# tongdaxu/VQ-VAE-from-Gaussian-VAE

Hardware: AMD Instinct MI355X
Metric: images/sec encode+quantize+decode, 256x256, codebook 2^16 (higher is better)
Workload: dtype f32

## Files before the change

vq-vae-from-gaussian-vae_amd/csrc/gq_wino_gemm.h:

```cpp
#pragma once
#include "gq_common.h"

namespace gqhip {

typedef _Float16 f16x8 __attribute__((ext_vector_type(8)));

struct WinoGemm2Params {
  const _Float16 *V2;
  const _Float16 *Wf;
  float *M;
  long tiles;
  int cin, cout, nnb;
  long mtiles;
  long ntile_total;
  long tiles_per_xcd;
};

__global__ __launch_bounds__(256, 2) void wino_gemm_f16x2_kernel(const WinoGemm2Params p) {
  constexpr int kPlane = 256 * 32 + 64, kChunk = 2 * kPlane, kStage = 2 * kChunk;
  __shared__ __attribute__((aligned(16))) unsigned char sA[2 * kStage];
  const int tid = threadIdx.x, lane = tid & 63, wave = __builtin_amdgcn_readfirstlane(tid >> 6);
  const int c = lane & 31, h = lane >> 5, wm = wave >> 1, wn = wave & 1;
  const long vb = blockIdx.x, kq = vb >> 3;
  const int nb = (int)(kq % p.nnb);
  const long tile = (vb & 7) * p.tiles_per_xcd + kq / p.nnb;
  if (tile >= p.ntile_total) return;
  const long pos = tile / p.mtiles, m0 = (tile % p.mtiles) * 256;
  const int cin = p.cin, nst = cin / 32;
  const int w8 = tid & 7, r0 = tid >> 3, pl = w8 >> 2, jc = (w8 >> 1) & 1, jh = w8 & 1;
  const _Float16 *src = p.V2 + ((pos * p.tiles + m0 + r0) * 2L * cin) + pl * cin + 16 * jc + 8 * jh;
  const int loff = jc * kChunk + pl * kPlane + r0 * 32 + 16 * (jh ^ ((r0 >> 3) & 1));
  const long rstride = 64L * cin;
  f16x8 st[8];
  auto issue = [&](int stage) {
#pragma unroll
    for (int i = 0; i < 8; ++i) st[i] = *reinterpret_cast<const f16x8 *>(src + i * rstride + stage * 32);
  };
  auto commit = [&](int buf) {
#pragma unroll
    for (int i = 0; i < 8; ++i) *reinterpret_cast<f16x8 *>(sA + buf * kStage + loff + i * 1024) = st[i];
  };
  f32x16 acc[4][2];
#pragma unroll
  for (int rr = 0; rr < 4; ++rr)
#pragma unroll
    for (int j = 0; j < 2; ++j)
      acc[rr][j] = f32x16{0.f, 0.f, 0.f, 0.f, 0.f, 0.f, 0.f, 0.f, 0.f, 0.f, 0.f, 0.f, 0.f, 0.f, 0.f, 0.f};
  const int aoff = (4 * wm) * 1024 + c * 32 + 16 * (h ^ ((c >> 3) & 1));
  const long wstep = (long)p.nnb * (512 * 16);
  const unsigned char *wbase = reinterpret_cast<const unsigned char *>(p.Wf) + pos * (cin / 16) * wstep +
                               (4 * nb + 2 * wn) * 128 * 16;
  const int wl = lane * 16;
  f16x8 b0[4], b1[4];
  auto load_b = [&](int ks, f16x8 (&dst)[4]) {
    const unsigned char *s = wbase + ks * wstep;
#pragma unroll
    for (int k = 0; k < 4; ++k) dst[k] = *reinterpret_cast<const f16x8 *>(s + k * 1024 + wl);
  };
  auto kstep = [&](const unsigned char *A, const f16x8 (&bq)[4]) {
#pragma unroll
    for (int rr = 0; rr < 4; ++rr) {
      const f16x8 ah = *reinterpret_cast<const f16x8 *>(A + aoff + rr * 1024);
      const f16x8 al = *reinterpret_cast<const f16x8 *>(A + aoff + rr * 1024 + kPlane);
#pragma unroll
      for (int j = 0; j < 2; ++j) {
        acc[rr][j] = __builtin_amdgcn_mfma_f32_32x32x16_f16(ah, bq[2 * j], acc[rr][j], 0, 0, 0);
        acc[rr][j] = __builtin_amdgcn_mfma_f32_32x32x16_f16(ah, bq[2 * j + 1], acc[rr][j], 0, 0, 0);
        acc[rr][j] = __builtin_amdgcn_mfma_f32_32x32x16_f16(al, bq[2 * j], acc[rr][j], 0, 0, 0);
      }
    }
  };
  const int nks = 2 * nst;
  load_b(0, b0);
  issue(0);
  commit(0);
  __syncthreads();
  for (int s = 0; s < nst; ++s) {
    const bool more = s + 1 < nst;
    const unsigned char *A = sA + (s & 1) * kStage;
    load_b(2 * s + 1, b1);
    if (more) issue(s + 1);
    kstep(A, b0);
    __builtin_amdgcn_sched_barrier(0);
    load_b(2 * s + 2 < nks ? 2 * s + 2 : nks - 1, b0);
    kstep(A + kChunk, b1);
    if (more) commit((s + 1) & 1);
    __builtin_amdgcn_sched_barrier(0);
    __syncthreads();
  }
  float *Mp = p.M + ((pos * p.tiles + m0 + 4 * wm * 32 + 4 * h) * (long)p.cout) + nb * 128 + c;
  const long cs = p.cout;
#pragma unroll
  for (int rr = 0; rr < 4; ++rr)
#pragma unroll
    for (int j = 0; j < 2; ++j) {
      float *base = Mp + (rr * 32L) * cs + (2 * wn + j) * 32;
#pragma unroll
      for (int r = 0; r < 16; ++r) base[(long)((r & 3) + 8 * (r >> 2)) * cs] = acc[rr][j][r];
    }
}

__global__ __launch_bounds__(512, 1) void wino_gemm_f16x2_w8_kernel(const WinoGemm2Params p) {
  constexpr int kPlane = 256 * 32 + 32, kChunk = 2 * kPlane, kStage = 4 * kChunk;
  static_assert(kChunk % 256 == 64 && kPlane % 256 == 32, "region stagger");
  __shared__ __attribute__((aligned(16))) unsigned char sA[2 * kStage];
  const int tid = threadIdx.x, lane = tid & 63, wave = __builtin_amdgcn_readfirstlane(tid >> 6);
  const int c = lane & 31, h = lane >> 5, wm = wave >> 2, wn = wave & 3;
  const long vb = blockIdx.x, kq = vb >> 3;
  const int nb = (int)(kq % p.nnb);
  const long tile = (vb & 7) * p.tiles_per_xcd + kq / p.nnb;
  if (tile >= p.ntile_total) return;
  const long pos = tile / p.mtiles, m0 = (tile % p.mtiles) * 256;
  const int cin = p.cin, nst = cin / 64;
  const int w16 = tid & 15, r0 = tid >> 4, pl = w16 >> 3, jc = (w16 >> 1) & 3, jh = w16 & 1;
  const _Float16 *src = p.V2 + ((pos * p.tiles + m0 + r0) * 2L * cin) + pl * cin + 16 * jc + 8 * jh;
  const int loff = jc * kChunk + pl * kPlane + r0 * 32 + 16 * (jh ^ ((r0 >> 3) & 1));
  const long rstride = 64L * cin;
  f16x8 st[8];
  auto issue = [&](int stage) {
#pragma unroll
    for (int i = 0; i < 8; ++i) st[i] = *reinterpret_cast<const f16x8 *>(src + i * rstride + stage * 64);
  };
  auto commit = [&](int buf) {
#pragma unroll
    for (int i = 0; i < 8; ++i) *reinterpret_cast<f16x8 *>(sA + buf * kStage + loff + i * 1024) = st[i];
  };
  f32x16 acc[4][2];
#pragma unroll
  for (int rr = 0; rr < 4; ++rr)
#pragma unroll
    for (int j = 0; j < 2; ++j)
      acc[rr][j] = f32x16{0.f, 0.f, 0.f, 0.f, 0.f, 0.f, 0.f, 0.f, 0.f, 0.f, 0.f, 0.f, 0.f, 0.f, 0.f, 0.f};
  const int aoff = (4 * wm) * 1024 + c * 32 + 16 * (h ^ ((c >> 3) & 1));
  const long wstep = (long)(p.cout / 32) * 2048;
  const unsigned char *wbase = reinterpret_cast<const unsigned char *>(p.Wf) + pos * (cin / 16) * wstep +
                               (8 * nb + 2 * wn) * 2048L;
  const int wl = lane * 16;
  const int nks = 4 * nst;
  f16x8 bA[4], bB[4], bC[4];
  auto load_b = [&](int ks, f16x8 (&dst)[4]) {
    const unsigned char *s = wbase + (long)(ks < nks ? ks : nks - 1) * wstep;
#pragma unroll
    for (int k = 0; k < 4; ++k) dst[k] = *reinterpret_cast<const f16x8 *>(s + k * 1024 + wl);
  };
  f16x8 ah, al, nh, nl;
  auto read_a = [&](const unsigned char *A, int u, f16x8 &oh, f16x8 &ol) {
    const unsigned char *q = A + (u >> 2) * kChunk + aoff + (u & 3) * 1024;
    oh = *reinterpret_cast<const f16x8 *>(q);
    ol = *reinterpret_cast<const f16x8 *>(q + kPlane);
  };
  auto mfma6 = [&](int rr, const f16x8 (&bq)[4]) {
#pragma unroll
    for (int j = 0; j < 2; ++j) {
      acc[rr][j] = __builtin_amdgcn_mfma_f32_32x32x16_f16(ah, bq[2 * j], acc[rr][j], 0, 0, 0);
      acc[rr][j] = __builtin_amdgcn_mfma_f32_32x32x16_f16(ah, bq[2 * j + 1], acc[rr][j], 0, 0, 0);
      acc[rr][j] = __builtin_amdgcn_mfma_f32_32x32x16_f16(al, bq[2 * j], acc[rr][j], 0, 0, 0);
    }
  };
  auto kstep = [&](const unsigned char *A, int ks4, const f16x8 (&bq)[4], bool last_of_stage) {
#pragma unroll
    for (int rr = 0; rr < 4; ++rr) {
      const int u = 4 * ks4 + rr;
      if (!(last_of_stage && rr == 3)) read_a(A, u + 1, nh, nl);
      __builtin_amdgcn_sched_barrier(0);
      mfma6(rr, bq);
      ah = nh;
      al = nl;
      __builtin_amdgcn_sched_barrier(0);
    }
  };
  load_b(0, bA);
  load_b(1, bB);
  issue(0);
  commit(0);
  __syncthreads();
  for (int s = 0; s < nst; ++s) {
    const bool more = s + 1 < nst;
    const unsigned char *A = sA + (s & 1) * kStage;
    read_a(A, 0, ah, al);
    load_b(4 * s + 2, bC);
    if (more) issue(s + 1);
    kstep(A, 0, bA, false);
    load_b(4 * s + 3, bA);
    kstep(A, 1, bB, false);
    load_b(4 * s + 4, bB);
    kstep(A, 2, bC, false);
    load_b(4 * s + 5, bC);
    kstep(A, 3, bA, true);
    if (more) commit((s + 1) & 1);
#pragma unroll
    for (int k = 0; k < 4; ++k) {
      bA[k] = bB[k];
      bB[k] = bC[k];
    }
    __builtin_amdgcn_sched_barrier(0);
    __syncthreads();
  }
  float *Mp = p.M + ((pos * p.tiles + m0 + 4 * wm * 32 + 4 * h) * (long)p.cout) + nb * 256 + c;
  const long cs = p.cout;
#pragma unroll
  for (int rr = 0; rr < 4; ++rr)
#pragma unroll
    for (int j = 0; j < 2; ++j) {
      float *base = Mp + (rr * 32L) * cs + (2 * wn + j) * 32;
#pragma unroll
      for (int r = 0; r < 16; ++r) base[(long)((r & 3) + 8 * (r >> 2)) * cs] = acc[rr][j][r];
    }
}

}
```

Before: 489.5.

## Switch Winograd GEMM kernels to 16x16x32 MFMA with transposed operands

```diff
diff --git a/vq-vae-from-gaussian-vae_amd/csrc/gq_wino_gemm.h b/vq-vae-from-gaussian-vae_amd/csrc/gq_wino_gemm.h
--- a/vq-vae-from-gaussian-vae_amd/csrc/gq_wino_gemm.h
+++ b/vq-vae-from-gaussian-vae_amd/csrc/gq_wino_gemm.h
@@ -20,7 +20,7 @@
   constexpr int kPlane = 256 * 32 + 64, kChunk = 2 * kPlane, kStage = 2 * kChunk;
   __shared__ __attribute__((aligned(16))) unsigned char sA[2 * kStage];
   const int tid = threadIdx.x, lane = tid & 63, wave = __builtin_amdgcn_readfirstlane(tid >> 6);
-  const int c = lane & 31, h = lane >> 5, wm = wave >> 1, wn = wave & 1;
+  const int c = lane & 15, g = lane >> 4, wm = wave >> 1, wn = wave & 1;
   const long vb = blockIdx.x, kq = vb >> 3;
   const int nb = (int)(kq % p.nnb);
   const long tile = (vb & 7) * p.tiles_per_xcd + kq / p.nnb;
@@ -40,64 +40,59 @@
 #pragma unroll
     for (int i = 0; i < 8; ++i) *reinterpret_cast<f16x8 *>(sA + buf * kStage + loff + i * 1024) = st[i];
   };
-  f32x16 acc[4][2];
+  f32x4 acc[8][4];
 #pragma unroll
-  for (int rr = 0; rr < 4; ++rr)
+  for (int m = 0; m < 8; ++m)
 #pragma unroll
-    for (int j = 0; j < 2; ++j)
-      acc[rr][j] = f32x16{0.f, 0.f, 0.f, 0.f, 0.f, 0.f, 0.f, 0.f, 0.f, 0.f, 0.f, 0.f, 0.f, 0.f, 0.f, 0.f};
-  const int aoff = (4 * wm) * 1024 + c * 32 + 16 * (h ^ ((c >> 3) & 1));
+    for (int n = 0; n < 4; ++n) acc[m][n] = f32x4{0.f, 0.f, 0.f, 0.f};
+  const int aoff = (g >> 1) * kChunk + (8 * wm) * 512 + c * 32 + 16 * ((g & 1) ^ ((c >> 3) & 1));
   const long wstep = (long)p.nnb * (512 * 16);
   const unsigned char *wbase = reinterpret_cast<const unsigned char *>(p.Wf) + pos * (cin / 16) * wstep +
-                               (4 * nb + 2 * wn) * 128 * 16;
-  const int wl = lane * 16;
-  f16x8 b0[4], b1[4];
-  auto load_b = [&](int ks, f16x8 (&dst)[4]) {
-    const unsigned char *s = wbase + ks * wstep;
+                               (4 * nb + 2 * wn) * 128 * 16 + (g >> 1) * wstep + (32 * (g & 1) + c) * 16;
+  f16x8 wH[4], wN[4], wL[4];
+  auto load_w = [&](int ks, int plane, f16x8 (&dst)[4]) {
+    const unsigned char *s = wbase + (long)(ks < nst ? ks : nst - 1) * 2 * wstep + plane * 1024;
 #pragma unroll
-    for (int k = 0; k < 4; ++k) dst[k] = *reinterpret_cast<const f16x8 *>(s + k * 1024 + wl);
+    for (int n = 0; n < 4; ++n) dst[n] = *reinterpret_cast<const f16x8 *>(s + (n >> 1) * 2048 + (n & 1) * 256);
   };
-  auto kstep = [&](const unsigned char *A, const f16x8 (&bq)[4]) {
+  auto products = [&](const unsigned char *A, int plane) {
 #pragma unroll
-    for (int rr = 0; rr < 4; ++rr) {
-      const f16x8 ah = *reinterpret_cast<const f16x8 *>(A + aoff + rr * 1024);
-      const f16x8 al = *reinterpret_cast<const f16x8 *>(A + aoff + rr * 1024 + kPlane);
+    for (int m = 0; m < 8; ++m) {
+      const f16x8 a = *reinterpret_cast<const f16x8 *>(A + plane * kPlane + aoff + m * 512);
 #pragma unroll
-      for (int j = 0; j < 2; ++j) {
-        acc[rr][j] = __builtin_amdgcn_mfma_f32_32x32x16_f16(ah, bq[2 * j], acc[rr][j], 0, 0, 0);
-        acc[rr][j] = __builtin_amdgcn_mfma_f32_32x32x16_f16(ah, bq[2 * j + 1], acc[rr][j], 0, 0, 0);
-        acc[rr][j] = __builtin_amdgcn_mfma_f32_32x32x16_f16(al, bq[2 * j], acc[rr][j], 0, 0, 0);
+      for (int n = 0; n < 4; ++n) acc[m][n] = __builtin_amdgcn_mfma_f32_16x16x32_f16(wH[n], a, acc[m][n], 0, 0, 0);
+      if (plane == 0) {
+#pragma unroll
+        for (int n = 0; n < 4; ++n) acc[m][n] = __builtin_amdgcn_mfma_f32_16x16x32_f16(wL[n], a, acc[m][n], 0, 0, 0);
       }
     }
   };
-  const int nks = 2 * nst;
-  load_b(0, b0);
+  load_w(0, 0, wH);
+  load_w(0, 1, wL);
   issue(0);
   commit(0);
   __syncthreads();
   for (int s = 0; s < nst; ++s) {
     const bool more = s + 1 < nst;
     const unsigned char *A = sA + (s & 1) * kStage;
-    load_b(2 * s + 1, b1);
+    load_w(s + 1, 0, wN);
     if (more) issue(s + 1);
-    kstep(A, b0);
+    products(A, 0);
     __builtin_amdgcn_sched_barrier(0);
-    load_b(2 * s + 2 < nks ? 2 * s + 2 : nks - 1, b0);
-    kstep(A + kChunk, b1);
+    load_w(s + 1, 1, wL);
+    products(A, 1);
     if (more) commit((s + 1) & 1);
+#pragma unroll
+    for (int n = 0; n < 4; ++n) wH[n] = wN[n];
     __builtin_amdgcn_sched_barrier(0);
     __syncthreads();
   }
-  float *Mp = p.M + ((pos * p.tiles + m0 + 4 * wm * 32 + 4 * h) * (long)p.cout) + nb * 128 + c;
+  float *Mp = p.M + ((pos * p.tiles + m0 + 8 * wm * 16 + c) * (long)p.cout) + nb * 128 + wn * 64 + 4 * g;
   const long cs = p.cout;
 #pragma unroll
-  for (int rr = 0; rr < 4; ++rr)
+  for (int m = 0; m < 8; ++m)
 #pragma unroll
-    for (int j = 0; j < 2; ++j) {
-      float *base = Mp + (rr * 32L) * cs + (2 * wn + j) * 32;
-#pragma unroll
-      for (int r = 0; r < 16; ++r) base[(long)((r & 3) + 8 * (r >> 2)) * cs] = acc[rr][j][r];
-    }
+    for (int n = 0; n < 4; ++n) *reinterpret_cast<f32x4 *>(Mp + (m * 16L) * cs + n * 16) = acc[m][n];
 }
 
 __global__ __launch_bounds__(512, 1) void wino_gemm_f16x2_w8_kernel(const WinoGemm2Params p) {
@@ -105,7 +100,7 @@
   static_assert(kChunk % 256 == 64 && kPlane % 256 == 32, "region stagger");
   __shared__ __attribute__((aligned(16))) unsigned char sA[2 * kStage];
   const int tid = threadIdx.x, lane = tid & 63, wave = __builtin_amdgcn_readfirstlane(tid >> 6);
-  const int c = lane & 31, h = lane >> 5, wm = wave >> 2, wn = wave & 3;
+  const int c = lane & 15, g = lane >> 4, wm = wave >> 2, wn = wave & 3;
   const long vb = blockIdx.x, kq = vb >> 3;
   const int nb = (int)(kq % p.nnb);
   const long tile = (vb & 7) * p.tiles_per_xcd + kq / p.nnb;
@@ -125,87 +120,69 @@
 #pragma unroll
     for (int i = 0; i < 8; ++i) *reinterpret_cast<f16x8 *>(sA + buf * kStage + loff + i * 1024) = st[i];
   };
-  f32x16 acc[4][2];
+  f32x4 acc[8][4];
 #pragma unroll
-  for (int rr = 0; rr < 4; ++rr)
+  for (int m = 0; m < 8; ++m)
 #pragma unroll
-    for (int j = 0; j < 2; ++j)
-      acc[rr][j] = f32x16{0.f, 0.f, 0.f, 0.f, 0.f, 0.f, 0.f, 0.f, 0.f, 0.f, 0.f, 0.f, 0.f, 0.f, 0.f, 0.f};
-  const int aoff = (4 * wm) * 1024 + c * 32 + 16 * (h ^ ((c >> 3) & 1));
+    for (int n = 0; n < 4; ++n) acc[m][n] = f32x4{0.f, 0.f, 0.f, 0.f};
+  const int aoff = (g >> 1) * kChunk + (8 * wm) * 512 + c * 32 + 16 * ((g & 1) ^ ((c >> 3) & 1));
   const long wstep = (long)(p.cout / 32) * 2048;
   const unsigned char *wbase = reinterpret_cast<const unsigned char *>(p.Wf) + pos * (cin / 16) * wstep +
-                               (8 * nb + 2 * wn) * 2048L;
-  const int wl = lane * 16;
-  const int nks = 4 * nst;
-  f16x8 bA[4], bB[4], bC[4];
-  auto load_b = [&](int ks, f16x8 (&dst)[4]) {
-    const unsigned char *s = wbase + (long)(ks < nks ? ks : nks - 1) * wstep;
+                               (8 * nb + 2 * wn) * 2048L + (g >> 1) * wstep + (32 * (g & 1) + c) * 16;
+  const int nk32 = 2 * nst;
+  f16x8 wH0[4], wH1[4], wL[4], aq[4];
+  auto load_w = [&](int ks, int plane, f16x8 (&dst)[4]) {
+    const unsigned char *s = wbase + (long)(ks < nk32 ? ks : nk32 - 1) * 2 * wstep + plane * 1024;
 #pragma unroll
-    for (int k = 0; k < 4; ++k) dst[k] = *reinterpret_cast<const f16x8 *>(s + k * 1024 + wl);
+    for (int n = 0; n < 4; ++n) dst[n] = *reinterpret_cast<const f16x8 *>(s + (n >> 1) * 2048 + (n & 1) * 256);
   };
-  f16x8 ah, al, nh, nl;
-  auto read_a = [&](const unsigned char *A, int u, f16x8 &oh, f16x8 &ol) {
-    const unsigned char *q = A + (u >> 2) * kChunk + aoff + (u & 3) * 1024;
-    oh = *reinterpret_cast<const f16x8 *>(q);
-    ol = *reinterpret_cast<const f16x8 *>(q + kPlane);
+  auto read_a = [&](const unsigned char *A, int u, f16x8 &o) {
+    o = *reinterpret_cast<const f16x8 *>(A + (u >> 4) * 2 * kChunk + ((u >> 3) & 1) * kPlane + aoff + (u & 7) * 512);
   };
-  auto mfma6 = [&](int rr, const f16x8 (&bq)[4]) {
+  auto unit = [&](int u, const f16x8 &a, const f16x8 (&wh)[4], const f16x8 (&wl)[4]) {
+    const int m = u & 7;
 #pragma unroll
-    for (int j = 0; j < 2; ++j) {
-      acc[rr][j] = __builtin_amdgcn_mfma_f32_32x32x16_f16(ah, bq[2 * j], acc[rr][j], 0, 0, 0);
-      acc[rr][j] = __builtin_amdgcn_mfma_f32_32x32x16_f16(ah, bq[2 * j + 1], acc[rr][j], 0, 0, 0);
-      acc[rr][j] = __builtin_amdgcn_mfma_f32_32x32x16_f16(al, bq[2 * j], acc[rr][j], 0, 0, 0);
+    for (int n = 0; n < 4; ++n) acc[m][n] = __builtin_amdgcn_mfma_f32_16x16x32_f16(wh[n], a, acc[m][n], 0, 0, 0);
+    if (((u >> 3) & 1) == 0) {
+#pragma unroll
+      for (int n = 0; n < 4; ++n) acc[m][n] = __builtin_amdgcn_mfma_f32_16x16x32_f16(wl[n], a, acc[m][n], 0, 0, 0);
     }
   };
-  auto kstep = [&](const unsigned char *A, int ks4, const f16x8 (&bq)[4], bool last_of_stage) {
-#pragma unroll
-    for (int rr = 0; rr < 4; ++rr) {
-      const int u = 4 * ks4 + rr;
-      if (!(last_of_stage && rr == 3)) read_a(A, u + 1, nh, nl);
-      __builtin_amdgcn_sched_barrier(0);
-      mfma6(rr, bq);
-      ah = nh;
-      al = nl;
-      __builtin_amdgcn_sched_barrier(0);
-    }
-  };
-  load_b(0, bA);
-  load_b(1, bB);
+  load_w(0, 0, wH0);
+  load_w(0, 1, wL);
+  load_w(1, 0, wH1);
   issue(0);
   commit(0);
   __syncthreads();
   for (int s = 0; s < nst; ++s) {
     const bool more = s + 1 < nst;
     const unsigned char *A = sA + (s & 1) * kStage;
-    read_a(A, 0, ah, al);
-    load_b(4 * s + 2, bC);
+    read_a(A, 0, aq[0]);
+    read_a(A, 1, aq[1]);
+    read_a(A, 2, aq[2]);
     if (more) issue(s + 1);
-    kstep(A, 0, bA, false);
-    load_b(4 * s + 3, bA);
-    kstep(A, 1, bB, false);
-    load_b(4 * s + 4, bB);
-    kstep(A, 2, bC, false);
-    load_b(4 * s + 5, bC);
-    kstep(A, 3, bA, true);
+#pragma unroll
+    for (int u = 0; u < 32; ++u) {
+      if (u + 3 < 32) read_a(A, u + 3, aq[(u + 3) & 3]);
+      __builtin_amdgcn_sched_barrier(0);
+      if (u < 16) unit(u, aq[u & 3], wH0, wL);
+      else unit(u, aq[u & 3], wH1, wL);
+      __builtin_amdgcn_sched_barrier(0);
+      if (u == 7) load_w(2 * s + 1, 1, wL);
+      if (u == 15) load_w(2 * s + 2, 0, wH0);
+      if (u == 23) load_w(2 * s + 2, 1, wL);
+      if (u == 31) load_w(2 * s + 3, 0, wH1);
+    }
     if (more) commit((s + 1) & 1);
-#pragma unroll
-    for (int k = 0; k < 4; ++k) {
-      bA[k] = bB[k];
-      bB[k] = bC[k];
-    }
     __builtin_amdgcn_sched_barrier(0);
     __syncthreads();
   }
-  float *Mp = p.M + ((pos * p.tiles + m0 + 4 * wm * 32 + 4 * h) * (long)p.cout) + nb * 256 + c;
+  float *Mp = p.M + ((pos * p.tiles + m0 + 8 * wm * 16 + c) * (long)p.cout) + nb * 256 + wn * 64 + 4 * g;
   const long cs = p.cout;
 #pragma unroll
-  for (int rr = 0; rr < 4; ++rr)
+  for (int m = 0; m < 8; ++m)
 #pragma unroll
-    for (int j = 0; j < 2; ++j) {
-      float *base = Mp + (rr * 32L) * cs + (2 * wn + j) * 32;
-#pragma unroll
-      for (int r = 0; r < 16; ++r) base[(long)((r & 3) + 8 * (r >> 2)) * cs] = acc[rr][j][r];
-    }
+    for (int n = 0; n < 4; ++n) *reinterpret_cast<f32x4 *>(Mp + (m * 16L) * cs + n * 16) = acc[m][n];
 }
 
 }
```

New measurement: 490.3, median of 6. Within noise of the previous version (+0.2%).
